# MDIL-SNU/SevenNet

Hardware: NVIDIA H100
Metric: atom_updates_per_sec (higher is better)
Workload: dtype f32

## Files before the change

sevenn_b200/csrc/common.cuh:

```cuda
#pragma once
#include <cuda_runtime.h>
#include <cstdint>
#include <cstdio>

#include "vec_ops.cuh"

namespace s7b {

constexpr float kSiluNorm = 1.6791767923989418f;
constexpr int kMaxPaths = 12;
constexpr int kMaxL = 4;

S7B_HD float silu_n(float z) {
  const float s = 1.0f / (1.0f + expf(-z));
  return kSiluNorm * z * s;
}
S7B_HD float dsilu_n(float z) {
  const float s = 1.0f / (1.0f + expf(-z));
  return kSiluNorm * s * (1.0f + z * (1.0f - s));
}

struct ConvRole {
  int x_off;
  int mul;
  int tab_off;
  int w_off[kMaxPaths];
  int out_off[kMaxPaths];
  int out_stride[kMaxPaths];
};

__host__ __device__ constexpr int y_stride(int ny) { return (ny - 1 + 3) / 4 * 4; }

constexpr int kConvWrongMul = 3;
constexpr int kConvNoPath = 4;

struct ConvArgs {
  const int* rowptr;
  const int4* rec;
  const float* Y;
  const float* x;
  const float4* table;
  const uint2* table23;
  const float* w;
  int n_begin, n_dst;
  int dim_x, dim_mid, w_numel;
  float inv_h;
  unsigned int* row_max;
  int rows_per_node;
};

}

#define S7B_CUDA_CHECK(expr)                                                            \
  do {                                                                                  \
    cudaError_t _e = (expr);                                                            \
    if (_e != cudaSuccess) {                                                            \
      s7b::set_error(__FILE__, __LINE__, cudaGetErrorString(_e));                       \
      return 1;                                                                         \
    }                                                                                   \
  } while (0)

namespace s7b {
void set_error(const char* file, int line, const char* msg);
}
```

sevenn_b200/csrc/conv_kernels.cuh:

```cuda
#pragma once
#include <cuda_fp16.h>

#include "common.cuh"
#include "generated/tp_kinds.cuh"

namespace s7b {

constexpr int kConvWarpsPerBlock = 4;
constexpr int kConvMul[kMaxL] = {128, 64, 32, 32};
constexpr int kConvMaxMul = 1024;

template <int MUL>
__device__ __forceinline__ int conv_mul(const ConvRole& role) {
  if constexpr (MUL > 0) return MUL;
  else return role.mul;
}
#ifndef S7B_FWD_MINBLOCKS
#define S7B_FWD_MINBLOCKS 1
#endif
#define S7B_FWD_BOUNDS __launch_bounds__(32 * kConvWarpsPerBlock, S7B_FWD_MINBLOCKS)
#ifdef S7B_BWD_MINBLOCKS
#define S7B_BWD_BOUNDS __launch_bounds__(32 * kConvWarpsPerBlock, S7B_BWD_MINBLOCKS)
#else
#define S7B_BWD_BOUNDS __launch_bounds__(32 * kConvWarpsPerBlock, \
    (Kind::NY != 9 || (MUL == 0 && Kind::D1 > 1)) ? 2 : ((Kind::D1 == 3 || !NEED_DX) ? 4 : 3))
#endif
#ifndef S7B_COOP_REC
#define S7B_COOP_REC 1
#endif

template <int LPN>
struct EdgeRecs {
  int cx, cy, cz;
  __device__ __forceinline__ void fill(const ConvArgs& a, int e0, int len, int it, int sl) {
    const int ei = it + sl;
    int4 r = make_int4(0, 0, 0, 0);
    if (ei < len) r = __ldg(a.rec + (unsigned)(e0 + ei));
    cx = r.x; cy = r.y; cz = r.z;
  }
  __device__ __forceinline__ int4 get(int it) const {
    const int l = it % LPN;
    return make_int4(__shfl_sync(0xffffffffu, cx, l, LPN), __shfl_sync(0xffffffffu, cy, l, LPN),
                     __shfl_sync(0xffffffffu, cz, l, LPN), 0);
  }
};

template <int M, int LPN>
__device__ __forceinline__ void group_reduce_multi(float (&v)[M], int sl) {
  static_assert((M == 8 || M == 16) && (LPN == 16 || LPN == 32) && M <= LPN, "unsupported reduction shape");
  int off = LPN / 2;
#pragma unroll
  for (int m = M / 2; m >= 1; m >>= 1, off >>= 1) {
    const bool up = (sl & off) != 0;
#pragma unroll
    for (int j = 0; j < m; ++j) {
      const float send = up ? v[j] : v[j + m];
      const float keep = up ? v[j + m] : v[j];
      v[j] = keep + __shfl_xor_sync(0xffffffffu, send, off);
    }
  }
#pragma unroll
  for (; off >= 1; off >>= 1) v[0] += __shfl_xor_sync(0xffffffffu, v[0], off);
}

template <int LPN>
__device__ __forceinline__ float group_sum(float v) {
#pragma unroll
  for (int off = LPN / 2; off >= 1; off >>= 1) v += __shfl_xor_sync(0xffffffffu, v, off);
  return v;
}

template <class Kind>
__device__ __forceinline__ void load_Y(const float* __restrict__ Yrow, float (&Y)[Kind::NY]) {
  Y[0] = 1.0f;
  constexpr int NQ = (Kind::NY - 1 + 3) / 4;
  const float4* p = reinterpret_cast<const float4*>(Yrow);
#pragma unroll
  for (int q = 0; q < NQ; ++q) {
    const float4 v = __ldg(p + q);
    if (4 * q + 1 < Kind::NY) Y[4 * q + 1] = v.x;
    if (4 * q + 2 < Kind::NY) Y[4 * q + 2] = v.y;
    if (4 * q + 3 < Kind::NY) Y[4 * q + 3] = v.z;
    if (4 * q + 4 < Kind::NY) Y[4 * q + 4] = v.w;
  }
}

__device__ __forceinline__ size_t row_offset(int i, int stride) { return (size_t)(unsigned)i * (unsigned)stride; }

__device__ __forceinline__ float2 ldg2(const float* p) { return __ldg(reinterpret_cast<const float2*>(p)); }

template <class V> struct VT;
template <> struct VT<V2> {
  static constexpr int CH = 2;
  static __device__ __forceinline__ V2 zero() { return splat2(0.0f); }
  static __device__ __forceinline__ V2 load(const float* p) { return ldg2(p); }
  static __device__ __forceinline__ void store(float* p, V2 v) { *reinterpret_cast<float2*>(p) = v; }
  static __device__ __forceinline__ float hsum(V2 v) { return v.x + v.y; }
  static __device__ __forceinline__ float amax(V2 v) { return fmaxf(fabsf(v.x), fabsf(v.y)); }
  static __device__ __forceinline__ void coef(const float4* t01, const uint2* t23, bool, V2& a0, V2& a1, V2& a2, V2& a3) {
    const float4 c01 = __ldg(t01);
    const uint2 c23 = __ldg(t23);
    a0 = make_float2(c01.x, c01.y);
    a1 = make_float2(c01.z, c01.w);
    a2 = __half22float2(*reinterpret_cast<const __half2*>(&c23.x));
    a3 = __half22float2(*reinterpret_cast<const __half2*>(&c23.y));
  }
};
template <> struct VT<float> {
  static constexpr int CH = 1;
  static __device__ __forceinline__ float zero() { return 0.0f; }
  static __device__ __forceinline__ float load(const float* p) { return __ldg(p); }
  static __device__ __forceinline__ void store(float* p, float v) { *p = v; }
  static __device__ __forceinline__ float hsum(float v) { return v; }
  static __device__ __forceinline__ float amax(float v) { return fabsf(v); }
  static __device__ __forceinline__ void coef(const float4* t01, const uint2* t23, bool odd, float& a0, float& a1, float& a2, float& a3) {
    const float4 c01 = __ldg(t01);
    const uint2 c23 = __ldg(t23);
    const float2 h2 = __half22float2(*reinterpret_cast<const __half2*>(&c23.x));
    const float2 h3 = __half22float2(*reinterpret_cast<const __half2*>(&c23.y));
    a0 = odd ? c01.y : c01.x;
    a1 = odd ? c01.w : c01.z;
    a2 = odd ? h2.y : h2.x;
    a3 = odd ? h3.y : h3.x;
  }
};

template <int NV, int LPN, int CH>
struct LaneMap {
  int n, sl, uc0, e0, len, nmax;
  bool node_ok;
  __device__ __forceinline__ LaneMap(const ConvArgs& a) {
    constexpr int GPW = 32 / LPN;
    const int lane = threadIdx.x & 31;
    sl = lane % LPN;
    n = a.n_begin + (blockIdx.x * kConvWarpsPerBlock + (threadIdx.x >> 5)) * GPW + lane / LPN;
    node_ok = n < a.n_dst;
    uc0 = blockIdx.y * (CH * LPN * NV) + CH * sl;
    e0 = 0;
    len = 0;
    if (node_ok) {
      e0 = __ldg(a.rowptr + n);
      len = __ldg(a.rowptr + n + 1) - e0;
    }
    nmax = len;
    if (GPW > 1) nmax = max(len, __shfl_xor_sync(0xffffffffu, len, 16));
  }
};

template <class Kind, int MUL, int NV, int LPN, bool TABLE, class V>
__global__ void S7B_FWD_BOUNDS
conv_fwd_kernel(const ConvArgs a, const ConvRole role, float* __restrict__ out) {
  constexpr int CH = VT<V>::CH;
  static_assert(MUL % (CH * LPN * NV) == 0, "channels must fill whole lane groups");
  const int mul = conv_mul<MUL>(role);
  const LaneMap<NV, LPN, CH> m(a);
  if (m.nmax == 0 && !m.node_ok) return;

  V acc[NV][Kind::NACC];
#pragma unroll
  for (int c = 0; c < NV; ++c)
#pragma unroll
    for (int q = 0; q < Kind::NACC; ++q) acc[c][q] = VT<V>::zero();

  const unsigned xlane = role.x_off + m.uc0;
  const unsigned tlane = role.tab_off + (m.uc0 >> 1);
  const bool odd = (m.uc0 & 1) != 0;
  EdgeRecs<LPN> recs;
  for (int it = 0; it < m.nmax; ++it) {
    const bool valid = (LPN == 32) || (it < m.len);
    const int e = valid ? m.e0 + it : 0;
#if S7B_COOP_REC
    if (it % LPN == 0) recs.fill(a, m.e0, m.len, it, m.sl);
    const int4 rec = recs.get(it);
#else
    const int4 rec = __ldg(a.rec + e);
#endif
    float Y[Kind::NY];
    load_Y<Kind>(a.Y + row_offset(e, y_stride(Kind::NY)), Y);
    const float* __restrict__ xrow = a.x + (row_offset(rec.x, a.dim_x) + xlane);
    const unsigned ti = tlane + rec.y * (Kind::NPATH * mul / 2);
    const float4* __restrict__ k01 = a.table + ti;
    const uint2* __restrict__ k23 = a.table23 + ti;
    const float tt = __int_as_float(rec.z);
#pragma unroll
    for (int c = 0; c < NV; ++c) {
      const int u = CH * LPN * c;
      V x[Kind::D1], w[Kind::NPATH];
#pragma unroll
      for (int i = 0; i < Kind::D1; ++i) x[i] = VT<V>::load(xrow + i * mul + u);
#pragma unroll
      for (int p = 0; p < Kind::NPATH; ++p) {
        if (TABLE) {
          V a0, a1, a2, a3;
          VT<V>::coef(k01 + (p * (mul / 2) + u / 2), k23 + (p * (mul / 2) + u / 2), odd, a0, a1, a2, a3);
          w[p] = fma_(tt, fma_(tt, fma_(tt, a3, a2), a1), a0);
        } else {
          w[p] = VT<V>::load(a.w + (size_t)e * a.w_numel + role.w_off[p] + m.uc0 + u);
        }
        if (LPN != 32 && !valid) w[p] = VT<V>::zero();
      }
      Kind::fwd(x, Y, w, acc[c]);
    }
  }

  if (a.row_max != nullptr) {
#pragma unroll
    for (int l3 = 0; l3 < kMaxL; ++l3) {
      bool present = false;
#pragma unroll
      for (int p = 0; p < Kind::NPATH; ++p) present = present || (Kind::path_l3(p) == l3);
      if (!present) continue;
#pragma unroll
      for (int k = 0; k < 2 * l3 + 1; ++k) {
        float mx = 0.0f;
#pragma unroll
        for (int c = 0; c < NV; ++c)
#pragma unroll
          for (int p = 0; p < Kind::NPATH; ++p)
            if (Kind::path_l3(p) == l3) mx = fmaxf(mx, VT<V>::amax(acc[c][Kind::acc_off(p) + k]));
#pragma unroll
        for (int off = LPN / 2; off >= 1; off >>= 1) mx = fmaxf(mx, __shfl_xor_sync(0xffffffffu, mx, off));
        if (m.node_ok && m.sl == 0) atomicMax(a.row_max + (size_t)m.n * a.rows_per_node + l3 * l3 + k, __float_as_uint(mx));
      }
    }
  }
  if (!m.node_ok) return;
  float* __restrict__ orow = out + (size_t)m.n * a.dim_mid;
#pragma unroll
  for (int c = 0; c < NV; ++c) {
    const int u = m.uc0 + CH * LPN * c;
#pragma unroll
    for (int p = 0; p < Kind::NPATH; ++p) {
#pragma unroll
      for (int k = 0; k < 2 * Kind::path_l3(p) + 1; ++k)
        VT<V>::store(orow + role.out_off[p] + k * role.out_stride[p] + u, acc[c][Kind::acc_off(p) + k]);
    }
// ... 114 lines not shown
```

sevenn_b200/csrc/edge_kernels.cuh:

```cuda
#pragma once
#include "common.cuh"
#include "generated/sh.cuh"

namespace s7b {

struct RadialDesc {
  float cutoff;
  int cutoff_fn;
  float cutoff_on;
  int poly_p;
  int n_basis;
  float coeffs[8];
  float inv_h;
  int knots;
};

S7B_HD void envelope(const RadialDesc& d, float r, float& env, float& denv) {
  if (d.cutoff_fn == 0) {
    if (r < d.cutoff_on) { env = 1.0f; denv = 0.0f; return; }
    const float r2 = r * r, on2 = d.cutoff_on * d.cutoff_on, c2 = d.cutoff * d.cutoff;
    const float den = (c2 - on2) * (c2 - on2) * (c2 - on2);
    const float a = c2 - r2, b = c2 + 2.0f * r2 - 3.0f * on2;
    env = a * a * b / den;
    denv = (-4.0f * r * a * b + 4.0f * r * a * a) / den;
  } else {
    const float p = (float)d.poly_p;
    const float x = r / d.cutoff;
    float xp = 1.0f;
    for (int i = 0; i < d.poly_p - 1; ++i) xp *= x;
    const float c0 = (p + 1.0f) * (p + 2.0f) * 0.5f, c1 = p * (p + 2.0f), c2 = p * (p + 1.0f) * 0.5f;
    env = 1.0f - xp * x * (c0 - c1 * x + c2 * x * x);
    denv = -xp * (c0 * p - c1 * (p + 1.0f) * x + c2 * (p + 2.0f) * x * x) / d.cutoff;
  }
}

template <int LMAX>
__global__ void edge_fwd_kernel(const RadialDesc rd, const float* __restrict__ edge_vec,
                                const int* __restrict__ src, const int64_t* __restrict__ n_edges_p, int ny_stride,
                                int4* __restrict__ rec, float* __restrict__ Yout,
                                float* __restrict__ rlen, float* __restrict__ emb) {
  const int64_t e = (int64_t)blockIdx.x * blockDim.x + threadIdx.x;
  if (e >= *n_edges_p) return;
  const float vx = edge_vec[3 * e], vy = edge_vec[3 * e + 1], vz = edge_vec[3 * e + 2];
  const float r = sqrtf(vx * vx + vy * vy + vz * vz);
  const float ir = r > 0.0f ? 1.0f / r : 0.0f;
  float Y[SH<LMAX>::NY];
  SH<LMAX>::eval(vx * ir, vy * ir, vz * ir, Y);
  float* yrow = Yout + e * ny_stride;
#pragma unroll
  for (int j = 1; j < SH<LMAX>::NY; ++j) yrow[j - 1] = Y[j];
  for (int j = SH<LMAX>::NY - 1; j < ny_stride; ++j) yrow[j] = 0.0f;
  const float s = r * rd.inv_h;
  int tk = (int)s;
  tk = tk < 0 ? 0 : (tk > rd.knots - 1 ? rd.knots - 1 : tk);
  const float tt = fminf(fmaxf(s - (float)tk, 0.0f), 1.0f);
  rec[e] = make_int4(__ldg(src + e), tk, __float_as_int(tt), 0);
  rlen[e] = r;
  if (emb != nullptr) {
    float env, denv;
    envelope(rd, r, env, denv);
    const float pre = 2.0f / rd.cutoff;
    for (int b = 0; b < rd.n_basis; ++b) emb[e * rd.n_basis + b] = pre * sinf(rd.coeffs[b] * r) * ir * env;
  }
}

template <int LMAX>
__global__ void edge_bwd_kernel(const RadialDesc rd, const float* __restrict__ edge_vec,
                                const int64_t* __restrict__ n_edges_p, int64_t part_stride, int ny_stride, int n_part,
                                const float* __restrict__ dY_acc, const float* __restrict__ dEdr_acc,
                                const float* __restrict__ demb, float* __restrict__ fedge) {
  const int64_t e = (int64_t)blockIdx.x * blockDim.x + threadIdx.x;
  if (e >= *n_edges_p) return;
  const float vx = edge_vec[3 * e], vy = edge_vec[3 * e + 1], vz = edge_vec[3 * e + 2];
  const float r = sqrtf(vx * vx + vy * vy + vz * vz);
  const float ir = r > 0.0f ? 1.0f / r : 0.0f;
  const float ux = vx * ir, uy = vy * ir, uz = vz * ir;
  float gY[SH<LMAX>::NY];
  gY[0] = 0.0f;
#pragma unroll
  for (int j = 1; j < SH<LMAX>::NY; ++j) gY[j] = 0.0f;
  float gr = 0.0f;
  for (int p = 0; p < n_part; ++p) {
    const float* row = dY_acc + ((size_t)p * part_stride + e) * ny_stride;
#pragma unroll
    for (int j = 1; j < SH<LMAX>::NY; ++j) gY[j] += row[j - 1];
    if (dEdr_acc != nullptr) gr += dEdr_acc[(size_t)p * part_stride + e];
  }
  if (demb != nullptr) {
    float env, denv;
// ... 73 lines not shown
```

sevenn_b200/csrc/engine.cu:

```cuda
#include <algorithm>
#include <cstdlib>
#include <cstring>
#include <functional>
#include <map>
#include <string>
#include <vector>

#include "../../include/sevenn_b200.h"
#include "common.cuh"
#include "conv_kernels.cuh"
#include "edge_kernels.cuh"
#include "neighbor.cuh"
#include "node_kernels.cuh"
#include "tc_gemm.cuh"

namespace s7b {

static thread_local std::string g_error;
static int64_t g_launches = 0;
extern int64_t g_conv_launches;

void set_error(const char* file, int line, const char* msg) {
  char buf[512];
  snprintf(buf, sizeof(buf), "%s:%d: %s", file, line, msg);
// ... 69 lines not shown
      pool.push_back(r.b);
    }
    recs.clear();
  }
  void clear() { collect(); totals.clear(); }
};

struct ProfScope {
  Profiler* p;
  cudaStream_t st;
  cudaEvent_t b;
  ProfScope(Profiler& prof, cudaStream_t s, const char* what, int t = -1, int l = -1) : p(nullptr), st(s) {
    if (!prof.enabled) return;
    p = &prof;
    char buf[64];
    if (t >= 0 && l >= 0) snprintf(buf, sizeof(buf), "%s.t%d.l%d", what, t, l);
    else if (t >= 0) snprintf(buf, sizeof(buf), "%s.t%d", what, t);
    else snprintf(buf, sizeof(buf), "%s", what);
    cudaEvent_t a = prof.get();
    b = prof.get();
    cudaEventRecord(a, st);
    prof.recs.push_back({buf, a, b});
  }
  ~ProfScope() { if (p) cudaEventRecord(b, st); }
};

struct LayerCfg {
  int n_lx = 0, n_lg = 0;
  int x_muls[kMaxL] = {0}, out_muls[kMaxL] = {0}, g_muls[kMaxL] = {0};
  int x_off[kMaxL] = {0}, g_off[kMaxL] = {0}, h_off[kMaxL] = {0};
  int dim_x = 0, dim_g = 0, dim_h = 0, dim_mid = 0, W = 0;
  int mid_K[kMaxL] = {0}, mid_off[kMaxL] = {0};
  int lmax_out = 0;
  std::vector<PathCfg> paths;
  ConvRole roles[kMaxL];
  GateDesc gate;
  std::map<std::string, DevBuf> params;
  std::map<std::string, struct TcWeights*> tcw;
};

struct RowExp {
  DevBuf buf;
  int rows_per_node = 0;
  bool bits = false;
};

}

using namespace s7b;

struct S7bEngine {
  S7bModelDesc desc;
  std::vector<LayerCfg> layers;
  std::map<std::string, DevBuf> params;
  RadialDesc radial;
  bool radial_ready = false;
  int ny_stride = 8;
  int n_nodes = 0, n_local = 0, n_interior = 0;
  int64_t n_edges = 0;
  const int* d_species = nullptr;
  const int* d_rowptr = nullptr;
  const int* d_src = nullptr;
  const float* d_edge_vec = nullptr;
  DevBuf rec, Y, rlen, emb, dY_acc, dEdr_acc, demb_acc, fedge;
  std::vector<DevBuf> x, g, wbuf, z1, z2, h1, h2;
  DevBuf mid, h, dh, dg, dx, dwbuf, tmpA, tmpB;
// ... 496 lines not shown
  return irreps_linear(A, lda, a_off, a_K, C, ldc, c_off, c_N, n_l, W, n_nodes, accumulate, st);
}

static int dense_gemm(const float* A, int K, float* C, int N, const float* W, int64_t rows, int epilogue,
                      const float* aux_in, float* aux_out, bool accumulate, cudaStream_t st) {
  const int64_t chunk = 1 << 22;
  for (int64_t r0 = 0; r0 < rows; r0 += chunk) {
    const int n = (int)std::min<int64_t>(chunk, rows - r0);
    LinArgs a;
    memset(&a, 0, sizeof(a));
    a.A = A + r0 * K;
    a.C = C + r0 * N;
    a.aux_in = aux_in ? aux_in + r0 * N : nullptr;
    a.aux_out = aux_out ? aux_out + r0 * N : nullptr;
    a.lda = K;
    a.ldc = N;
    a.n_nodes = n;
    a.accumulate = accumulate ? 1 : 0;
    a.epilogue = epilogue;
    a.nblocks = 1;
    a.blk[0] = LinBlock{W, 1, K, N, 0, K, 0, N};
    if (launch_gemm(a, st)) return 1;
  }
  return 0;
}

static int conv_forward(const LayerCfg& L, int lmax_filter, bool table, ConvArgs a, float* out,
                        cudaStream_t st) {
  for (int l1 = 0; l1 < L.n_lx; ++l1)
    if (launch_conv_fwd(l1, lmax_filter, L.lmax_out, table, a, L.roles[l1], out, st)) return 1;
  return 0;
}

static std::vector<float> role_table_images(const LayerCfg& L, int knots, const float* host, int floats_per_pair) {
  std::vector<float> img((size_t)knots * (L.W / 2) * floats_per_pair);
  for (int l1 = 0; l1 < L.n_lx; ++l1) {
    const ConvRole& r = L.roles[l1];
    std::vector<int> cols;
    for (const PathCfg& q : L.paths)
      if (q.l1 == l1) cols.push_back(q.w_off);
    const size_t run = (size_t)(r.mul / 2) * floats_per_pair;
    float* dst = img.data() + (size_t)r.tab_off * floats_per_pair;
    for (int k = 0; k < knots; ++k)
      for (int c : cols) {
        memcpy(dst, host + ((size_t)k * (L.W / 2) + c / 2) * floats_per_pair, run * sizeof(float));
        dst += run;
      }
  }
  return img;
}

}

extern "C" {

const char* s7b_last_error(void) { return g_error.c_str(); }
int s7b_version(void) { return 1; }
int64_t s7b_launch_count(int reset) {
  const int64_t v = g_launches + g_conv_launches;
  if (reset) { g_launches = 0; g_conv_launches = 0; }
  return v;
}

int s7b_set_option(const char* name, int value) {
  if (!name) return fail("null option name");
  if (std::string(name) == "tc_gemm") { g_opt_tc_gemm = value; return 0; }
  if (std::string(name) == "tc_swizzle") { g_opt_tc_swizzle = value; return 0; }
  if (std::string(name) == "atomic_virial") { g_opt_atomic_virial = value; return 0; }
  if (std::string(name) == "concurrent_conv") { g_opt_concurrent = value; return 0; }
  if (std::string(name) == "cuda_graph") { g_opt_cuda_graph = value; return 0; }
  if (std::string(name) == "stage_graphs") { g_opt_stage_graphs = value; return 0; }
  if (std::string(name) == "gate_bwd_rows") { g_opt_gate_bwd_rows = value; return 0; }
  return fail(std::string("unknown option: ") + name);
}

int s7b_gather_rows(const float* src, int32_t ld_src, const int32_t* idx, int64_t n, int32_t width, float* out, void* stream) {
// ... 238 lines not shown
    DevBuf& dst = e->layers[layer].params[nm];
    if (dst.ensure(numel * sizeof(float))) return fail("cudaMalloc failed for parameter " + nm);
    S7B_CUDA_CHECK(cudaMemcpy(dst.p, host, numel * sizeof(float), cudaMemcpyHostToDevice));
    if (!e->species_sc) {
      e->species_sc = true;
      if (e->seg.ensure((2 * (size_t)S + 2) * sizeof(int)) || e->seg_perm.ensure((size_t)std::max(e->n_local, 1) * sizeof(int)))
        return fail("cudaMalloc failed for the species segmentation");
      ++g_alloc_gen;
    }
    return 0;
  }
  if (layer >= 0 && (nm == "sc" || nm == "scT") && layer < e->desc.n_layers &&
      (e->layers[layer].params.count("sc_species") || e->layers[layer].params.count("scT_species")))
    return fail("layer " + std::to_string(layer) + ": parameter " + nm + " and the species-wise self-connection 'sc_species' / 'scT_species' cannot both be set");
  if (nm == "bessel") {
    if ((int)numel != e->desc.n_basis) return fail("bessel: wrong size");
    for (int b = 0; b < e->desc.n_basis; ++b) e->radial.coeffs[b] = host[b];
    e->radial_ready = true;
    return 0;
  }
  DevBuf* dst;
  if (layer < 0) dst = &e->params[nm];
  else {
    if (layer >= e->desc.n_layers) return fail("layer out of range");
    dst = &e->layers[layer].params[nm];
  }
  std::vector<float> img;
  if (layer >= 0 && (nm == "table" || nm == "table23")) {
    const int fpp = nm == "table" ? 4 : 2;
    const LayerCfg& L = e->layers[layer];
    if (e->desc.table_knots <= 0) return fail("parameter " + nm + ": the model was created without radial tables");
    if (numel != (size_t)e->desc.table_knots * (L.W / 2) * fpp)
      return fail("parameter " + nm + ": size does not match the layer configuration and knot count");
    img = role_table_images(L, e->desc.table_knots, host, fpp);
    host = img.data();
  }
  if (dst->ensure(numel * sizeof(float))) return fail("cudaMalloc failed for parameter " + nm);
  S7B_CUDA_CHECK(cudaMemcpy(dst->p, host, numel * sizeof(float), cudaMemcpyHostToDevice));
  if (layer >= 0 && (nm == "si1" || nm == "si1T" || nm == "sc" || nm == "scT" || nm == "si2" || nm == "si2T")) {
    LayerCfg& L = e->layers[layer];
    int Ks[kMaxL] = {0, 0, 0, 0}, Ns[kMaxL] = {0, 0, 0, 0}, n_l = 0;
    const bool T = nm.back() == 'T';
    if (nm.rfind("si1", 0) == 0) { n_l = L.n_lx; for (int l = 0; l < n_l; ++l) { Ks[l] = L.x_muls[l]; Ns[l] = L.x_muls[l]; } }
    else if (nm.rfind("sc", 0) == 0) { n_l = std::min(L.n_lx, L.n_lg); for (int l = 0; l < n_l; ++l) { Ks[l] = L.x_muls[l]; Ns[l] = L.g_muls[l]; } }
    else { n_l = L.n_lg; for (int l = 0; l < n_l; ++l) { Ks[l] = L.mid_K[l]; Ns[l] = L.g_muls[l]; } }
    if (T) for (int l = 0; l < n_l; ++l) std::swap(Ks[l], Ns[l]);
    size_t expect = 0;
    for (int l = 0; l < n_l; ++l) expect += (size_t)Ks[l] * Ns[l];
    if (expect != numel) return fail("parameter " + nm + ": size does not match the layer configuration");
    TcWeights*& w = L.tcw[nm];
    if (!w) w = new TcWeights();
    if (tc_build_weights(*w, host, Ks, Ns, n_l)) return 1;
    ++g_alloc_gen;
  }
  return 0;
}

static const float* lparam(const S7bEngine* e, int t, const char* name) {
  auto it = e->layers[t].params.find(name);
  return it == e->layers[t].params.end() ? nullptr : it->second.as<float>();
}
static const float* gparam(const S7bEngine* e, const char* name) {
  auto it = e->params.find(name);
  return it == e->params.end() ? nullptr : it->second.as<float>();
}

int s7b_engine_set_graph(S7bEngine* e, int32_t n_nodes, int32_t n_local, int64_t n_edges,
                         const int32_t* d_species, const int32_t* d_rowptr, const int32_t* d_src,
// ... 64 lines not shown
  rc |= e->energy.ensure(sizeof(double));
  rc |= e->virial.ensure(6 * sizeof(double));
  rc |= e->atomic_energy.ensure(Nl * sizeof(float));
  rc |= e->atomic_energy64.ensure(Nl * sizeof(double));
  rc |= e->forces.ensure(Nn * 3 * sizeof(float));
  if (e->want_atomic_virial) rc |= e->atomic_virial.ensure(Nn * 6 * sizeof(float));
  if (rc) return fail("cudaMalloc failed while sizing step buffers");
  return 0;
}

int s7b_engine_set_interior(S7bEngine* e, int32_t n_interior) {
  if (!e) return fail("null engine");
  if (n_interior < 0 || n_interior > e->n_local) return fail("n_interior out of range");
  e->n_interior = n_interior;
  return 0;
}

static ConvArgs make_conv_args(const S7bEngine* e, int t, const float* x) {
  const LayerCfg& L = e->layers[t];
  ConvArgs a;
  memset(&a, 0, sizeof(a));
  a.rowptr = e->d_rowptr;
  a.rec = e->rec.as<int4>();
  a.Y = e->Y.as<float>();
  a.x = x;
  a.table = reinterpret_cast<const float4*>(lparam(e, t, "table"));
  a.table23 = reinterpret_cast<const uint2*>(lparam(e, t, "table23"));
  a.w = e->desc.table_knots > 0 ? nullptr : e->wbuf[t].as<float>();
  a.n_dst = e->n_local;
  a.dim_x = L.dim_x;
  a.dim_mid = L.dim_mid;
  a.w_numel = L.W;
  a.inv_h = e->radial.inv_h;
  return a;
}

static int grid1d(size_t total, int block) {
  size_t g = (total + block - 1) / block;
  if (g > 132 * 64) g = 132 * 64;
  if (g < 1) g = 1;
  return (int)g;
}

static int require(const void* p, const char* what) {
  if (p) return 0;
  return fail(std::string("missing parameter: ") + what);
}

static int run_stage_impl(S7bEngine* e, int stage, int t, void* stream) {
  cudaStream_t st = reinterpret_cast<cudaStream_t>(stream);
  const int T = e->desc.n_layers;
  const int Nn = e->n_nodes, Nl = e->n_local;
  const int64_t E = e->n_edges;
  const int64_t Ecap = e->E_cap;
  const int64_t* nE = e->d_nE.as<int64_t>();
  const bool table = e->desc.table_knots > 0;
  const int LF = e->desc.lmax_filter;
  if (!e->radial_ready) return fail("parameter 'bessel' was not set");

  switch (stage) {
    case S7B_STAGE_FWD_BEGIN: {
      if (E > 0) {
        const int blk = 256;
        const int grd = (int)((Ecap + blk - 1) / blk);
        float* emb = table ? nullptr : e->emb.as<float>();
        ProfScope ps(e->prof, st, "edge_fwd");
// ... 13 lines not shown
      }
      const LayerCfg& L0 = e->layers[0];
      const float* ex = gparam(e, "embed_x0");
      const float* eg = gparam(e, "embed_g0");
      if (require(ex, "embed_x0") || require(eg, "embed_g0")) return 1;
      ProfScope ps(e->prof, st, "embed_gather");
      if (Nn > 0) {
        gather_rows_kernel<<<grid1d((size_t)Nn * L0.dim_x, 256), 256, 0, st>>>(ex, e->d_species, e->x[0].as<float>(), Nn, L0.dim_x, L0.dim_x);
        S7B_LAUNCH_CHECK();
      }
      if (Nl > 0) {
        gather_rows_kernel<<<grid1d((size_t)Nl * L0.dim_g, 256), 256, 0, st>>>(eg, e->d_species, e->g[0].as<float>(), Nl, L0.dim_g, L0.dim_g);
        S7B_LAUNCH_CHECK();
      }
      return 0;
    }
    case S7B_STAGE_FWD_LAYER:
    case S7B_STAGE_FWD_LAYER_A:
    case S7B_STAGE_FWD_CONV_INTERIOR:
    case S7B_STAGE_FWD_LAYER_A2: {
      if (t < 0 || t >= T) return fail("layer out of range");
      const LayerCfg& L = e->layers[t];
      if (Nl == 0) return 0;
      const bool head = stage != S7B_STAGE_FWD_LAYER_A2;
      if (head && !table && E > 0) {
        const float *w0 = lparam(e, t, "mlp0"), *w1 = lparam(e, t, "mlp1"), *w2 = lparam(e, t, "mlp2");
        if (require(w0, "mlp0") || require(w1, "mlp1") || require(w2, "mlp2")) return 1;
        const int nb = e->desc.n_basis, h0 = e->desc.radial_hidden[0], h1 = e->desc.radial_hidden[1];
        ProfScope ps(e->prof, st, "radial_mlp_fwd", t);
        if (dense_gemm(e->emb.as<float>(), nb, e->h1[t].as<float>(), h0, w0, E, kEpiSiluStoreZ, nullptr, e->z1[t].as<float>(), false, st)) return 1;
        if (dense_gemm(e->h1[t].as<float>(), h0, e->h2[t].as<float>(), h1, w1, E, kEpiSiluStoreZ, nullptr, e->z2[t].as<float>(), false, st)) return 1;
        if (dense_gemm(e->h2[t].as<float>(), h1, e->wbuf[t].as<float>(), L.W, w2, E, kEpiNone, nullptr, nullptr, false, st)) return 1;
      } else if (head && table) {
        if (require(lparam(e, t, "table"), "table") || require(lparam(e, t, "table23"), "table23")) return 1;
      }
      ConvArgs ca = make_conv_args(e, t, e->x[t].as<float>());
      if (stage == S7B_STAGE_FWD_CONV_INTERIOR) ca.n_dst = e->n_interior;
      if (stage == S7B_STAGE_FWD_LAYER_A2) ca.n_begin = e->n_interior;
      const bool fused_rows = g_opt_tc_gemm && L.tcw.count("si2") && L.tcw.at("si2") && L.tcw.at("si2")->ok;
      if (fused_rows) {
        e->re_mid.rows_per_node = L.n_lg * L.n_lg;
        e->re_mid.bits = true;
        if (head) S7B_CUDA_CHECK(cudaMemsetAsync(e->re_mid.buf.p, 0, (size_t)Nl * e->re_mid.rows_per_node * sizeof(int), st));
        ca.row_max = e->re_mid.buf.as<unsigned int>();
        ca.rows_per_node = e->re_mid.rows_per_node;
      }
      {
        const bool par = e->concurrent && g_opt_concurrent && !e->prof.enabled && L.n_lx > 1;
        if (par) S7B_CUDA_CHECK(cudaEventRecord(e->ev_fork, st));
        for (int l1 = 0; l1 < L.n_lx; ++l1) {
          cudaStream_t s1 = (par && l1 > 0) ? e->side[l1] : st;
          if (par && l1 > 0) S7B_CUDA_CHECK(cudaStreamWaitEvent(s1, e->ev_fork, 0));
          ProfScope ps(e->prof, s1, "conv_fwd", t, l1);
          if (launch_conv_fwd(l1, LF, L.lmax_out, table, ca, L.roles[l1], e->mid.as<float>(), s1)) return 1;
          if (par && l1 > 0) {
            S7B_CUDA_CHECK(cudaEventRecord(e->ev_join[l1], s1));
            S7B_CUDA_CHECK(cudaStreamWaitEvent(st, e->ev_join[l1], 0));
          }
        }
      }
      if (stage == S7B_STAGE_FWD_CONV_INTERIOR) return 0;
      const float* si2 = lparam(e, t, "si2");
      if (require(si2, "si2")) return 1;
      {
        ProfScope ps(e->prof, st, "si2_gemm", t);
        if (node_linear(L, "si2", e->re_mid, !fused_rows, L.n_lg, e->mid.as<float>(), L.dim_mid, L.mid_off, L.mid_K, e->g[t].as<float>(), L.dim_g, L.g_off, L.g_muls, L.n_lg, si2, Nl, true, st)) return 1;
      }
// ... 814 lines not shown
```

sevenn_b200/engine.py:

```python
from __future__ import annotations

import ctypes
import math
import os
from typing import Dict, Optional

import numpy as np

from .spec import SILU_NORM, ModelSpec, build_spec, check_sc_weight, sc_blocks

_LIB_PATH = os.environ.get('S7B_LIB') or os.path.join(os.path.dirname(os.path.abspath(__file__)), 'lib', 'libsevenn_b200.so')
_lib = None

S7B_MAX_LAYERS, S7B_MAX_L = 8, 4
(STAGE_FWD_BEGIN, STAGE_FWD_LAYER, STAGE_FWD_END, STAGE_BWD_LAYER_A, STAGE_BWD_LAYER_B,
 STAGE_BWD_END, STAGE_FWD_LAYER_A, STAGE_FWD_LAYER_SC, STAGE_BWD_LAYER_B1, STAGE_BWD_LAYER_B2,
 STAGE_FWD_CONV_INTERIOR, STAGE_FWD_LAYER_A2, STAGE_BWD_LAYER_A1, STAGE_BWD_LAYER_A2) = range(14)


class S7bModelDesc(ctypes.Structure):
    _fields_ = [
        ('n_layers', ctypes.c_int32), ('lmax_filter', ctypes.c_int32),
        ('num_species', ctypes.c_int32), ('n_basis', ctypes.c_int32),
        ('cutoff', ctypes.c_float), ('cutoff_fn', ctypes.c_int32),
# ... 130 lines not shown
        denv = np.where(r < spec.cutoff_on, 0.0, (-4 * r * a * b + 4 * r * a * a) / den)
    else:
        p = float(spec.poly_p)
        x = r / spec.cutoff
        env = 1 - (p + 1) * (p + 2) / 2 * x ** p + p * (p + 2) * x ** (p + 1) - p * (p + 1) / 2 * x ** (p + 2)
        denv = (-(p + 1) * (p + 2) / 2 * p * x ** (p - 1) + p * (p + 2) * (p + 1) * x ** p
                - p * (p + 1) / 2 * (p + 2) * x ** (p + 1)) / spec.cutoff
    return bes * env[:, None], dbes * env[:, None] + bes * denv[:, None]


def radial_weights(spec: ModelSpec, arrays: Dict[str, np.ndarray], t: int, r: np.ndarray):
    emb, demb = radial_embedding(spec, arrays['bessel_coeffs'], r)
    n_mlp = len(spec.radial_hidden) + 1
    h, dh = emb, demb
    for j in range(n_mlp):
        W = arrays[f'{t}.mlp{j}'].astype(np.float64) / math.sqrt(arrays[f'{t}.mlp{j}'].shape[0])
        z, dz = h @ W, dh @ W
        if j < n_mlp - 1:
            h, dh = SILU_NORM * _silu(z), SILU_NORM * _dsilu(z) * dz
        else:
            h, dh = z, dz
    return h, dh


def radial_table(spec: ModelSpec, arrays: Dict[str, np.ndarray], t: int, knots: int) -> np.ndarray:
    h = spec.cutoff / knots
    r = np.arange(knots + 1, dtype=np.float64) * h
    f, df = radial_weights(spec, arrays, t, r)
    f0, f1, d0, d1 = f[:-1], f[1:], df[:-1] * h, df[1:] * h
    tab = np.stack([f0, d0, 3 * (f1 - f0) - (2 * d0 + d1), 2 * (f0 - f1) + d0 + d1], axis=-1)
    return np.ascontiguousarray(tab, dtype=np.float32)


def pack_table_pairs(tab: np.ndarray):
    K, W, _ = tab.shape
    pairs = tab.reshape(K, W // 2, 2, 4)
    t01 = np.ascontiguousarray(pairs[..., 0:2].transpose(0, 1, 3, 2).reshape(K, W // 2, 4), dtype=np.float32)
    t23 = np.ascontiguousarray(pairs[..., 2:4].transpose(0, 1, 3, 2).reshape(K, W // 2, 4)).astype(np.float16)
    return t01, np.ascontiguousarray(t23).view(np.float32)


def default_table_knots(spec: ModelSpec) -> int:
    if spec.cutoff_fn != 'XPLOR':
        return 2048
    x = spec.cutoff_on / spec.cutoff
    dist = lambda n: abs(x * n - round(x * n))
    counts = range(2000, 4097)
    return next((n for n in counts if dist(n) < 1e-9), None) or min(counts, key=dist)


def prepare_params(spec: ModelSpec, arrays: Dict[str, np.ndarray], radial: str, knots: int):
    out: Dict[tuple, np.ndarray] = {}
    f64 = lambda a: np.asarray(a, dtype=np.float64)
    S = spec.num_species
    L0 = spec.layers[0]
    mul0 = L0.x_muls[0]
    h0 = f64(arrays['embed']).reshape(S, mul0) / math.sqrt(S)

    def lin_blocks(flat, in_muls, out_muls, n_l):
        blocks, off = [], 0
        for l in range(n_l):
            k, n = in_muls[l], out_muls[l]
            blocks.append(f64(flat[off:off + k * n]).reshape(k, n) / math.sqrt(k))
            off += k * n
        assert off == len(flat), (off, len(flat))
        return blocks
# ... 10 lines not shown
        t = L.t
        n_lx, n_lg = len(L.x_muls), len(L.gate_muls)
        si1 = lin_blocks(arrays[f'{t}.si1'], L.x_muls, L.x_muls, n_lx)
        n_sc = min(n_lx, n_lg)
        check_sc_weight(L, spec.self_connection, S, np.size(arrays[f'{t}.sc']))
        if nequip:
            sc = sc_species_blocks(arrays[f'{t}.sc'], L)
        else:
            sc = lin_blocks(arrays[f'{t}.sc'], L.x_muls, L.gate_muls, n_sc)
        den = float(arrays[f'{t}.den'][0])
        si2 = [b / den for b in lin_blocks(arrays[f'{t}.si2'], L.mid_K, L.gate_muls, n_lg)]
        if t == 0:
            x0 = h0 @ si1[0]
            g0 = np.zeros((S, L.dim_gate))
            if nequip:
                g0[:, :L.gate_muls[0]] = np.einsum('su,suw->sw', h0, sc[0])
            else:
                g0[:, :L.gate_muls[0]] = h0 @ sc[0]
            out[('embed_x0', -1)] = x0
            out[('embed_g0', -1)] = g0
        else:
            out[('si1', t)] = np.concatenate([b.ravel() for b in si1])
            out[('si1T', t)] = np.concatenate([b.T.ravel() for b in si1])
            if nequip:
                out[('sc_species', t)] = np.concatenate([b[s].ravel() for s in range(S) for b in sc])
                out[('scT_species', t)] = np.concatenate([b[s].T.ravel() for s in range(S) for b in sc])
            else:
                out[('sc', t)] = np.concatenate([b.ravel() for b in sc])
                out[('scT', t)] = np.concatenate([b.T.ravel() for b in sc])
        out[('si2', t)] = np.concatenate([b.ravel() for b in si2])
        out[('si2T', t)] = np.concatenate([b.T.ravel() for b in si2])
        if radial == 'table':
            out[('table', t)], out[('table23', t)] = pack_table_pairs(radial_table(spec, arrays, t, knots))
        else:
            for j in range(len(spec.radial_hidden) + 1):
                W = f64(arrays[f'{t}.mlp{j}'])
                W = W / math.sqrt(W.shape[0])
                out[(f'mlp{j}', t)] = W
                out[(f'mlp{j}T', t)] = W.T
    Lz = spec.layers[-1]
    r1 = f64(arrays['readout1']).reshape(Lz.out_muls[0], spec.readout_hidden) / math.sqrt(Lz.out_muls[0])
    r2 = f64(arrays['readout2']).reshape(spec.readout_hidden, 1) / math.sqrt(spec.readout_hidden)
    wr = (r1 @ r2).ravel()
    out[('readout', -1)] = wr
    out[('readout_lo', -1)] = wr - wr.astype(np.float32).astype(np.float64)
    out[('scale', -1)] = f64(arrays['scale'])
    out[('shift', -1)] = f64(arrays['shift'])
    out[('bessel', -1)] = f64(arrays['bessel_coeffs'])
    return {k: np.ascontiguousarray(v, dtype=np.float32) for k, v in out.items()}


def model_desc(spec: ModelSpec, knots: int) -> S7bModelDesc:
    d = S7bModelDesc()
    d.n_layers, d.lmax_filter, d.num_species, d.n_basis = spec.n_layers, spec.lmax_filter, spec.num_species, spec.n_basis
    d.cutoff, d.cutoff_fn = spec.cutoff, 0 if spec.cutoff_fn == 'XPLOR' else 1
    d.cutoff_on, d.poly_p = spec.cutoff_on, spec.poly_p
    if len(spec.radial_hidden) != 2:
        raise NotImplementedError('radial MLP must have two hidden layers')
    d.radial_hidden[0], d.radial_hidden[1] = spec.radial_hidden
    irreps = [list(L.x_muls) for L in spec.layers] + [list(spec.layers[-1].out_muls)]
    for t, muls in enumerate(irreps):
        d.n_l[t] = len(muls)
        for l, m in enumerate(muls):
            d.muls[t][l] = m
    d.table_knots = knots
    return d
# ... 289 lines not shown
```

Before: 1.771 million.

## Use dense linear value table for forward radial weights with cubic fallback for short edges

Adds a second forward-only radial table sampled at three times the knot density that stores corrected values, so the forward convolution does a linear interpolation from two float2 loads instead of reading four cubic coefficients. Edges shorter than a threshold radius are flagged during the first pass, and a second pass over the edges applies the original cubic table for them only when some lane in the warp saw one. This trades fewer coefficient bytes and FMAs per edge for a larger table, an extra radius field in the edge record, and a possible second edge loop. Accuracy now depends on the linear approximation of the radial function above the threshold.

```diff
diff --git a/sevenn_b200/csrc/common.cuh b/sevenn_b200/csrc/common.cuh
--- a/sevenn_b200/csrc/common.cuh
+++ b/sevenn_b200/csrc/common.cuh
@@ -27,6 +27,7 @@
   int w_off[kMaxPaths];
   int out_off[kMaxPaths];
   int out_stride[kMaxPaths];
+  int ftab_off;
 };
 
 __host__ __device__ constexpr int y_stride(int ny) { return (ny - 1 + 3) / 4 * 4; }
@@ -47,6 +48,9 @@
   float inv_h;
   unsigned int* row_max;
   int rows_per_node;
+  const float2* ftable;
+  float ftab_inv_h;
+  int ftab_knots;
 };
 
 }
diff --git a/sevenn_b200/csrc/conv_kernels.cuh b/sevenn_b200/csrc/conv_kernels.cuh
--- a/sevenn_b200/csrc/conv_kernels.cuh
+++ b/sevenn_b200/csrc/conv_kernels.cuh
@@ -28,6 +28,23 @@
 #ifndef S7B_COOP_REC
 #define S7B_COOP_REC 1
 #endif
+
+constexpr float kValueTableMinR = 0.6f;
+
+enum { kRecRaw = 0, kRecValue = 1, kRecCubicShort = 2 };
+template <int MODE>
+__device__ __forceinline__ int4 fwd_rec(const ConvArgs& a, int4 r, bool valid, bool& short_seen) {
+  const float rr = __int_as_float(r.w);
+  const bool is_short = valid && rr < kValueTableMinR;
+  if (MODE == kRecValue) {
+    short_seen = short_seen || is_short;
+    const int k = is_short ? a.ftab_knots - 1 : min(max((int)(rr * a.ftab_inv_h), 0), a.ftab_knots - 1);
+    const float t = is_short ? 1.0f : fminf(fmaxf(fmaf(rr, a.ftab_inv_h, -(float)k), 0.0f), 1.0f);
+    return make_int4(r.x, k, __float_as_int(t), 0);
+  }
+  if (MODE == kRecCubicShort) return make_int4(r.x, is_short ? r.y : ~r.y, r.z, 0);
+  return r;
+}
 
 template <int LPN>
 struct EdgeRecs {
@@ -38,6 +55,14 @@
     if (ei < len) r = __ldg(a.rec + (unsigned)(e0 + ei));
     cx = r.x; cy = r.y; cz = r.z;
   }
+  template <int MODE>
+  __device__ __forceinline__ void fill(const ConvArgs& a, int e0, int len, int it, int sl, bool& short_seen) {
+    const int ei = it + sl;
+    int4 r = make_int4(0, 0, 0, 0);
+    if (ei < len) r = __ldg(a.rec + (unsigned)(e0 + ei));
+    r = fwd_rec<MODE>(a, r, ei < len, short_seen);
+    cx = r.x; cy = r.y; cz = r.z;
+  }
   __device__ __forceinline__ int4 get(int it) const {
     const int l = it % LPN;
     return make_int4(__shfl_sync(0xffffffffu, cx, l, LPN), __shfl_sync(0xffffffffu, cy, l, LPN),
@@ -97,6 +122,7 @@
   static __device__ __forceinline__ void store(float* p, V2 v) { *reinterpret_cast<float2*>(p) = v; }
   static __device__ __forceinline__ float hsum(V2 v) { return v.x + v.y; }
   static __device__ __forceinline__ float amax(V2 v) { return fmaxf(fabsf(v.x), fabsf(v.y)); }
+  static __device__ __forceinline__ V2 val(const float2* p, bool) { return __ldg(p); }
   static __device__ __forceinline__ void coef(const float4* t01, const uint2* t23, bool, V2& a0, V2& a1, V2& a2, V2& a3) {
     const float4 c01 = __ldg(t01);
     const uint2 c23 = __ldg(t23);
@@ -113,6 +139,7 @@
   static __device__ __forceinline__ void store(float* p, float v) { *p = v; }
   static __device__ __forceinline__ float hsum(float v) { return v; }
   static __device__ __forceinline__ float amax(float v) { return fabsf(v); }
+  static __device__ __forceinline__ float val(const float2* p, bool odd) { return __ldg(reinterpret_cast<const float*>(p) + odd); }
   static __device__ __forceinline__ void coef(const float4* t01, const uint2* t23, bool odd, float& a0, float& a1, float& a2, float& a3) {
     const float4 c01 = __ldg(t01);
     const uint2 c23 = __ldg(t23);
@@ -147,40 +174,33 @@
   }
 };
 
-template <class Kind, int MUL, int NV, int LPN, bool TABLE, class V>
-__global__ void S7B_FWD_BOUNDS
-conv_fwd_kernel(const ConvArgs a, const ConvRole role, float* __restrict__ out) {
+template <class Kind, int MUL, int NV, int LPN, bool TABLE, class V, int MODE>
+__device__ __forceinline__ void conv_fwd_edges(const ConvArgs& a, const ConvRole& role,
+                                               const LaneMap<NV, LPN, VT<V>::CH>& m,
+                                               V (&acc)[NV][Kind::NACC], bool& short_seen) {
   constexpr int CH = VT<V>::CH;
-  static_assert(MUL % (CH * LPN * NV) == 0, "channels must fill whole lane groups");
   const int mul = conv_mul<MUL>(role);
-  const LaneMap<NV, LPN, CH> m(a);
-  if (m.nmax == 0 && !m.node_ok) return;
-
-  V acc[NV][Kind::NACC];
-#pragma unroll
-  for (int c = 0; c < NV; ++c)
-#pragma unroll
-    for (int q = 0; q < Kind::NACC; ++q) acc[c][q] = VT<V>::zero();
-
   const unsigned xlane = role.x_off + m.uc0;
-  const unsigned tlane = role.tab_off + (m.uc0 >> 1);
+  const unsigned tlane = (MODE == kRecCubicShort ? role.tab_off : role.ftab_off) + (m.uc0 >> 1);
   const bool odd = (m.uc0 & 1) != 0;
   EdgeRecs<LPN> recs;
   for (int it = 0; it < m.nmax; ++it) {
     const bool valid = (LPN == 32) || (it < m.len);
     const int e = valid ? m.e0 + it : 0;
 #if S7B_COOP_REC
-    if (it % LPN == 0) recs.fill(a, m.e0, m.len, it, m.sl);
+    if (it % LPN == 0) recs.template fill<MODE>(a, m.e0, m.len, it, m.sl, short_seen);
     const int4 rec = recs.get(it);
 #else
-    const int4 rec = __ldg(a.rec + e);
+    const int4 rec = fwd_rec<MODE>(a, __ldg(a.rec + e), valid, short_seen);
 #endif
     float Y[Kind::NY];
     load_Y<Kind>(a.Y + row_offset(e, y_stride(Kind::NY)), Y);
     const float* __restrict__ xrow = a.x + (row_offset(rec.x, a.dim_x) + xlane);
-    const unsigned ti = tlane + rec.y * (Kind::NPATH * mul / 2);
-    const float4* __restrict__ k01 = a.table + ti;
-    const uint2* __restrict__ k23 = a.table23 + ti;
+    const bool take = MODE != kRecCubicShort || rec.y >= 0;
+    const int k = take ? rec.y : ~rec.y;
+    const unsigned ti = tlane + k * (Kind::NPATH * mul / 2);
+    const float2* __restrict__ v0 = a.ftable + ti;
+    const float2* __restrict__ v1 = v0 + Kind::NPATH * mul / 2;
     const float tt = __int_as_float(rec.z);
 #pragma unroll
     for (int c = 0; c < NV; ++c) {
@@ -190,10 +210,14 @@
       for (int i = 0; i < Kind::D1; ++i) x[i] = VT<V>::load(xrow + i * mul + u);
 #pragma unroll
       for (int p = 0; p < Kind::NPATH; ++p) {
-        if (TABLE) {
+        if (MODE == kRecValue) {
+          const V w0 = VT<V>::val(v0 + (p * (mul / 2) + u / 2), odd);
+          const V w1 = VT<V>::val(v1 + (p * (mul / 2) + u / 2), odd);
+          w[p] = fma_(tt, w1, fma_(-tt, w0, w0));
+        } else if (MODE == kRecCubicShort) {
           V a0, a1, a2, a3;
-          VT<V>::coef(k01 + (p * (mul / 2) + u / 2), k23 + (p * (mul / 2) + u / 2), odd, a0, a1, a2, a3);
-          w[p] = fma_(tt, fma_(tt, fma_(tt, a3, a2), a1), a0);
+          VT<V>::coef(a.table + ti + (p * (mul / 2) + u / 2), a.table23 + ti + (p * (mul / 2) + u / 2), odd, a0, a1, a2, a3);
+          w[p] = take ? fma_(tt, fma_(tt, fma_(tt, a3, a2), a1), a0) : VT<V>::zero();
         } else {
           w[p] = VT<V>::load(a.w + (size_t)e * a.w_numel + role.w_off[p] + m.uc0 + u);
         }
@@ -202,6 +226,27 @@
       Kind::fwd(x, Y, w, acc[c]);
     }
   }
+}
+
+template <class Kind, int MUL, int NV, int LPN, bool TABLE, class V>
+__global__ void S7B_FWD_BOUNDS
+conv_fwd_kernel(const ConvArgs a, const ConvRole role, float* __restrict__ out) {
+  constexpr int CH = VT<V>::CH;
+  static_assert(MUL % (CH * LPN * NV) == 0, "channels must fill whole lane groups");
+  const LaneMap<NV, LPN, CH> m(a);
+  if (m.nmax == 0 && !m.node_ok) return;
+
+  V acc[NV][Kind::NACC];
+#pragma unroll
+  for (int c = 0; c < NV; ++c)
+#pragma unroll
+    for (int q = 0; q < Kind::NACC; ++q) acc[c][q] = VT<V>::zero();
+
+  bool short_seen = false;
+  conv_fwd_edges<Kind, MUL, NV, LPN, TABLE, V, TABLE ? kRecValue : kRecRaw>(a, role, m, acc, short_seen);
+  if constexpr (TABLE)
+    if (__any_sync(0xffffffffu, short_seen))
+      conv_fwd_edges<Kind, MUL, NV, LPN, TABLE, V, kRecCubicShort>(a, role, m, acc, short_seen);
 
   if (a.row_max != nullptr) {
 #pragma unroll
diff --git a/sevenn_b200/csrc/edge_kernels.cuh b/sevenn_b200/csrc/edge_kernels.cuh
--- a/sevenn_b200/csrc/edge_kernels.cuh
+++ b/sevenn_b200/csrc/edge_kernels.cuh
@@ -54,7 +54,7 @@
   int tk = (int)s;
   tk = tk < 0 ? 0 : (tk > rd.knots - 1 ? rd.knots - 1 : tk);
   const float tt = fminf(fmaxf(s - (float)tk, 0.0f), 1.0f);
-  rec[e] = make_int4(__ldg(src + e), tk, __float_as_int(tt), 0);
+  rec[e] = make_int4(__ldg(src + e), tk, __float_as_int(tt), __float_as_int(r));
   rlen[e] = r;
   if (emb != nullptr) {
     float env, denv;
diff --git a/sevenn_b200/csrc/engine.cu b/sevenn_b200/csrc/engine.cu
--- a/sevenn_b200/csrc/engine.cu
+++ b/sevenn_b200/csrc/engine.cu
@@ -125,6 +125,7 @@
   int dim_x = 0, dim_g = 0, dim_h = 0, dim_mid = 0, W = 0;
   int mid_K[kMaxL] = {0}, mid_off[kMaxL] = {0};
   int lmax_out = 0;
+  int ftab_knots = 0;
   std::vector<PathCfg> paths;
   ConvRole roles[kMaxL];
   GateDesc gate;
@@ -687,16 +688,18 @@
   return 0;
 }
 
-static std::vector<float> role_table_images(const LayerCfg& L, int knots, const float* host, int floats_per_pair) {
-  std::vector<float> img((size_t)knots * (L.W / 2) * floats_per_pair);
+static std::vector<float> role_table_images(const LayerCfg& L, int rows, const float* host, int floats_per_pair,
+                                            int* role_off) {
+  std::vector<float> img((size_t)rows * (L.W / 2) * floats_per_pair);
+  float* dst = img.data();
   for (int l1 = 0; l1 < L.n_lx; ++l1) {
     const ConvRole& r = L.roles[l1];
     std::vector<int> cols;
     for (const PathCfg& q : L.paths)
       if (q.l1 == l1) cols.push_back(q.w_off);
     const size_t run = (size_t)(r.mul / 2) * floats_per_pair;
-    float* dst = img.data() + (size_t)r.tab_off * floats_per_pair;
-    for (int k = 0; k < knots; ++k)
+    role_off[l1] = (int)((dst - img.data()) / floats_per_pair);
+    for (int k = 0; k < rows; ++k)
       for (int c : cols) {
         memcpy(dst, host + ((size_t)k * (L.W / 2) + c / 2) * floats_per_pair, run * sizeof(float));
         dst += run;
@@ -1001,8 +1004,25 @@
     if (e->desc.table_knots <= 0) return fail("parameter " + nm + ": the model was created without radial tables");
     if (numel != (size_t)e->desc.table_knots * (L.W / 2) * fpp)
       return fail("parameter " + nm + ": size does not match the layer configuration and knot count");
-    img = role_table_images(L, e->desc.table_knots, host, fpp);
+    int off[kMaxL];
+    img = role_table_images(L, e->desc.table_knots, host, fpp, off);
     host = img.data();
+  }
+  if (layer >= 0 && nm == "table_fwd") {
+    LayerCfg& L = e->layers[layer];
+    if (e->desc.table_knots <= 0) return fail("parameter " + nm + ": the model was created without radial tables");
+    const size_t rows = numel / (size_t)L.W;
+    if (numel % (size_t)L.W != 0 || rows < 2 || rows * (size_t)L.W / 2 > (size_t)INT32_MAX)
+      return fail("layer " + std::to_string(layer) + ": parameter table_fwd has " + std::to_string(numel) +
+                  " values, expected (knots + 1) x " + std::to_string(L.W) + " with at least one interval");
+    for (size_t c = 0; c < (size_t)L.W; ++c)
+      if (host[(rows - 1) * L.W + c] != 0.0f)
+        return fail("layer " + std::to_string(layer) + ": parameter table_fwd: the last knot (r = cutoff) must be 0");
+    int off[kMaxL];
+    img = role_table_images(L, (int)rows, host, 2, off);
+    host = img.data();
+    for (int l1 = 0; l1 < L.n_lx; ++l1) L.roles[l1].ftab_off = off[l1];
+    L.ftab_knots = (int)rows - 1;
   }
   if (dst->ensure(numel * sizeof(float))) return fail("cudaMalloc failed for parameter " + nm);
   S7B_CUDA_CHECK(cudaMemcpy(dst->p, host, numel * sizeof(float), cudaMemcpyHostToDevice));
@@ -1133,6 +1153,9 @@
   a.dim_mid = L.dim_mid;
   a.w_numel = L.W;
   a.inv_h = e->radial.inv_h;
+  a.ftable = reinterpret_cast<const float2*>(lparam(e, t, "table_fwd"));
+  a.ftab_knots = L.ftab_knots;
+  a.ftab_inv_h = L.ftab_knots > 0 ? (float)L.ftab_knots / e->desc.cutoff : 0.0f;
   return a;
 }
 
@@ -1212,7 +1235,8 @@
         if (dense_gemm(e->h1[t].as<float>(), h0, e->h2[t].as<float>(), h1, w1, E, kEpiSiluStoreZ, nullptr, e->z2[t].as<float>(), false, st)) return 1;
         if (dense_gemm(e->h2[t].as<float>(), h1, e->wbuf[t].as<float>(), L.W, w2, E, kEpiNone, nullptr, nullptr, false, st)) return 1;
       } else if (head && table) {
-        if (require(lparam(e, t, "table"), "table") || require(lparam(e, t, "table23"), "table23")) return 1;
+        if (require(lparam(e, t, "table"), "table") || require(lparam(e, t, "table23"), "table23") ||
+            require(lparam(e, t, "table_fwd"), "table_fwd")) return 1;
       }
       ConvArgs ca = make_conv_args(e, t, e->x[t].as<float>());
       if (stage == S7B_STAGE_FWD_CONV_INTERIOR) ca.n_dst = e->n_interior;
diff --git a/sevenn_b200/engine.py b/sevenn_b200/engine.py
--- a/sevenn_b200/engine.py
+++ b/sevenn_b200/engine.py
@@ -186,6 +186,30 @@
     return np.ascontiguousarray(tab, dtype=np.float32)
 
 
+def forward_table_knots(knots: int) -> int:
+    return 3 * knots
+
+
+def radial_value_table(spec: ModelSpec, arrays: Dict[str, np.ndarray], t: int, fknots: int) -> np.ndarray:
+    r = np.arange(fknots + 1, dtype=np.float64) * (spec.cutoff / fknots)
+    f, _ = radial_weights(spec, arrays, t, r)
+    d2 = np.zeros_like(f)
+    d2[1:-1] = f[2:] - 2.0 * f[1:-1] + f[:-2]
+    d2[0] = d2[1]
+    v = f - d2 / 12.0
+    v[-1] = 0.0
+    return np.ascontiguousarray(v, dtype=np.float32)
+
+
+def value_table_read(tab: np.ndarray, cutoff: float, r) -> np.ndarray:
+    K = tab.shape[0] - 1
+    inv_h = np.float32(np.float32(K) / np.float32(cutoff))
+    r32 = np.asarray(r, dtype=np.float32)
+    k = np.clip((r32 * inv_h).astype(np.int64), 0, K - 1)
+    t = np.clip((r32.astype(np.float64) * float(inv_h) - k).astype(np.float32), 0, 1).astype(np.float64)[:, None]
+    return (1.0 - t) * tab[k].astype(np.float64) + t * tab[k + 1].astype(np.float64)
+
+
 def pack_table_pairs(tab: np.ndarray):
     K, W, _ = tab.shape
     pairs = tab.reshape(K, W // 2, 2, 4)
@@ -262,6 +286,7 @@
         out[('si2T', t)] = np.concatenate([b.T.ravel() for b in si2])
         if radial == 'table':
             out[('table', t)], out[('table23', t)] = pack_table_pairs(radial_table(spec, arrays, t, knots))
+            out[('table_fwd', t)] = radial_value_table(spec, arrays, t, forward_table_knots(knots))
         else:
             for j in range(len(spec.radial_hidden) + 1):
                 W = f64(arrays[f'{t}.mlp{j}'])
```

Result: faster. 1.847 million, median of 6 (+4.3%).
